# MAGPIE-ICL/synthPy

Hardware: AMD Instinct MI355X
Metric: ray-steps/sec (+ rays/sec to detector), 1e7 rays x 512^3 volume (higher is better)
Workload: dtype f64

## Files before the change

synthpy_amd/csrc/trace_tile.inc:

```
struct TileGeom {
  int tb, tc;
  int halo;
  int band;
};

struct TileArgs {
  TraceArgs A;
  TileGeom G;
  int k0, k1;
  int first, last;
  int exit_rec, slab;
  int rot;
  unsigned block0;
  const double *rec_in;
  const uint32_t *order;
  uint32_t *perm_out;
  double *strag_rec;
  int64_t strag_cap;
  unsigned long long *strag_count;
};

constexpr int kRecColD = (1024 + 80) / 8;
__host__ __device__ constexpr int tile_rec(bool aux, bool rec = false) { return aux ? 38 : (rec ? 16 : 18); }

__host__ __device__ inline size_t tile_lds_bytes(const TileGeom &g, int seg_steps, bool aux = false, bool rec = false) {
  const size_t tables = (size_t)(2 * (g.tb + 1) + 2 * (g.tc + 1) + 4);
  (void)seg_steps;
  const size_t head = rec ? (((tables * sizeof(double)) + 1023) & ~(size_t)1023) / sizeof(double) : ((tables + 1) & ~(size_t)1);
  if (rec) return sizeof(double) * (head + (size_t)5 * g.tc * kRecColD);
  return sizeof(double) * (head + (size_t)5 * g.tb * g.tc * tile_rec(aux, rec));
}

__device__ __forceinline__ uint32_t band_key(int ib, int ic, int ncc, int band) {
  const int bnd = ib / band, row = ib - bnd * band;
  const int col = (bnd & 1) ? ncc - 1 - ic : ic;
  return ((uint32_t)bnd * (uint32_t)ncc + (uint32_t)col) * (uint32_t)band + (uint32_t)row;
}

__global__ void k_keys_band(VolDev V, const double *__restrict__ s0, int64_t N, int axis, int band, uint32_t oob_key, int shift,
                            uint32_t *__restrict__ keys) {
  const int64_t i = blockIdx.x * (int64_t)blockDim.x + threadIdx.x;
  if (i >= N) return;
  const int b = (axis + 1) % 3, c = (axis + 2) % 3;
  double pa = s0[axis * N + i], pb = s0[b * N + i], pc = s0[c * N + i];
  const double va = s0[(3 + axis) * N + i], vb = s0[(3 + b) * N + i], vc = s0[(3 + c) * N + i];
  const double ga0 = V.g[0][0];
  if (va > 0 && pa < ga0) {
    const double tau = (ga0 - pa) / va;
    pb = pb + vb * tau;
    pc = pc + vc * tau;
  }
  const double gb0 = V.g[1][0], gbL = V.g[1][V.nb - 1], gc0 = V.g[2][0], gcL = V.g[2][V.nc - 1];
  uint32_t key = oob_key;
  if (pb >= gb0 && pb <= gbL && pc >= gc0 && pc <= gcL) {
    const int ib = find_cell(V.g[1], V.nb, pb, gb0, (V.nb - 1) / (gbL - gb0));
    const int ic = find_cell(V.g[2], V.nc, pc, gc0, (V.nc - 1) / (gcL - gc0));
    key = band_key(ib, ic, V.nc - 1, band) >> shift;
  }
  keys[i] = key;
}

__global__ void k_keys_band_rec(VolDev V, const double *__restrict__ rec, int64_t N, int band, uint32_t oob_key, int shift,
                                uint32_t *__restrict__ keys) {
  const int64_t j = blockIdx.x * (int64_t)blockDim.x + threadIdx.x;
  if (j >= N) return;
  const double pb = rec[j], pc = rec[N + j], va = rec[2 * N + j];
  const double gb0 = V.g[1][0], gbL = V.g[1][V.nb - 1], gc0 = V.g[2][0], gcL = V.g[2][V.nc - 1];
  uint32_t key = oob_key;
  if (va > 0 && pb >= gb0 && pb <= gbL && pc >= gc0 && pc <= gcL) {
    const int ib = find_cell(V.g[1], V.nb, pb, gb0, (V.nb - 1) / (gbL - gb0));
    const int ic = find_cell(V.g[2], V.nc, pc, gc0, (V.nc - 1) / (gcL - gc0));
    key = band_key(ib, ic, V.nc - 1, band) >> shift;
  }
  keys[j] = key;
}

__global__ void k_strag_snap(const unsigned long long *count, unsigned long long *snap, int q, unsigned long long *total) {
  const unsigned long long c = *count;
  snap[q + 1] = c;
  *total += c - snap[q];
}

struct StragFinish {
  TraceArgs A;
  const double *strag;
  int64_t cap;
  int exit_rec, slab;
};
__global__ __launch_bounds__(256) void k_strag_finish(StragFinish F) {
  const TraceArgs &A = F.A;
  const int64_t N = A.N;
  const int64_t j = blockIdx.x * (int64_t)blockDim.x + threadIdx.x;
  const bool gone = j < N && A.rec[2 * N + j] == -__builtin_inf();
  double y[9];
#pragma unroll
  for (int row = 0; row < 9; ++row) y[row] = __builtin_nan("");
  if (gone) {
    const int64_t g = (int64_t)A.rec[j];
#pragma unroll
    for (int row = 0; row < 9; ++row) y[row] = F.strag[row * F.cap + g];
  }
  if (F.exit_rec) {
    if (gone) {
#pragma unroll
      for (int row = 0; row < 9; ++row) A.rec[row * N + j] = y[row];
    }
    return;
  }
  const bool finished = gone && y[2] == y[2] && y[6] <= A.t_end;
  if (finished) {
    const double rem = A.t_end - y[6];
    write_outputs(A, j, fma(y[2], rem, A.V.g[0][A.V.na - 1]), fma(y[3], rem, y[0]), fma(y[4], rem, y[1]), y[2], y[3], y[4], y[5], y[7], y[8]);
  }
  if (F.slab) {
    if (gone && !finished) write_lost(A, j);
  } else {
    queue_push(A.out_count, A.out_list, gone && !finished, (uint32_t)j);
  }
}

template <bool PHASE>
__global__ __launch_bounds__(256) void k_build_records(VolDev V, double *__restrict__ R) {
  const int64_t cells = (int64_t)(V.nb - 1) * (V.nc - 1), total = cells * V.na;
  for (int64_t t = blockIdx.x * (int64_t)blockDim.x + threadIdx.x; t < total; t += (int64_t)gridDim.x * blockDim.x) {
    const int k = (int)(t / cells);
    const int64_t rem = t - (int64_t)k * cells;
    const int ic = (int)(rem / (V.nb - 1)), ib = (int)(rem - (int64_t)ic * (V.nb - 1));
    const int64_t q = col8(V, ib, ic) + koff(V, k), sc = kSC, sb = (int64_t)V.nc * 8;
    float4 v[4] = {V.P[q], V.P[q + sc], V.P[q + sb], V.P[q + sb + sc]};
    float l[4] = {0.f, 0.f, 0.f, 0.f};
    if (PHASE) {
      l[0] = V.L[q];
      l[1] = V.L[q + sc];
      l[2] = V.L[q + sb];
      l[3] = V.L[q + sb + sc];
    }
    CoefPlane p;
    coefs_from_corners<PHASE>(v, l, p);
    double2 *o = reinterpret_cast<double2 *>(R + t * 16);
    o[0] = make_double2(p.a[0], p.a[1]);
    o[1] = make_double2(p.a[2], p.a[3]);
    o[2] = make_double2(p.b[0], p.b[1]);
    o[3] = make_double2(p.b[2], p.b[3]);
    o[4] = make_double2(p.c[0], p.c[1]);
    o[5] = make_double2(p.c[2], p.c[3]);
    o[6] = make_double2(p.d[0], p.d[1]);
    o[7] = make_double2(p.d[2], p.d[3]);
  }
}

#ifndef SR_TILE_THREADS
#define SR_TILE_THREADS 256
#endif
#ifndef SR_TILE_WAVES
#define SR_TILE_WAVES 3
#endif
#ifndef SR_TILE_REC_WAVES
#define SR_TILE_REC_WAVES 4
#endif
template <bool PHASE, bool AUX = false, bool REC = false>
__global__ __launch_bounds__(SR_TILE_THREADS, AUX ? 2 : (REC ? SR_TILE_REC_WAVES : SR_TILE_WAVES)) void k_trace_tile(TileArgs T) {
  static_assert(!(AUX && REC), "the ready-made records hold the gradient fields only");
  constexpr int kTileRec = tile_rec(AUX, REC);
  extern __shared__ double lds[];
  const TraceArgs &A = T.A;
  const VolDev &V = A.V;
  const int TB = T.G.tb, TC = T.G.tc, NC = TB * TC;
  double *tgb = lds, *trb = tgb + (TB + 1), *tgc = trb + (TB + 1), *trc = tgc + (TC + 1);
  int *org = reinterpret_cast<int *>(trc + (TC + 1));
  const size_t tables = REC ? ((((size_t)(2 * (TB + 1) + 2 * (TC + 1) + 4) * sizeof(double)) + 1023) & ~(size_t)1023) / sizeof(double)
                            : ((size_t)(2 * (TB + 1) + 2 * (TC + 1) + 4) + 1) & ~(size_t)1;
  double *recs = lds + tables;
  const int slot_d = REC ? TC * kRecColD : NC * kTileRec;
  auto cell_off = [&](int b_, int c_) { return REC ? c_ * (kRecColD * 8) + b_ * 16 : (c_ * TB + b_) * kTileRec; };

  const unsigned chunk = gridDim.x / 8;
  const unsigned bid = (blockIdx.x % 8) * chunk + blockIdx.x / 8;
  const bool wg_live = bid < A.n_blocks;
  const int64_t j = (int64_t)(T.block0 + bid) * blockDim.x + threadIdx.x;
  const bool have = wg_live && j < A.N;
  const int64_t N = A.N;
  const int a = A.axis, b = (a + 1) % 3, c = (a + 2) % 3;
  int64_t i = 0;

  double y0 = 0, y1 = 0, y2 = 1, y3 = 0, y4 = 0, y5 = 0, y6 = 0, y7 = 0, y8 = 0;
  bool alive = false;
  auto from_s0 = [&](const TraceArgs &Q, int64_t ray, double &q0, double &q1, double &q2, double &q3, double &q4, double &q5, double &q6) -> bool {
    const double pa = Q.s0[a * N + ray];
    q0 = Q.s0[b * N + ray];
    q1 = Q.s0[c * N + ray];
    q2 = Q.s0[(3 + a) * N + ray];
    q3 = Q.s0[(3 + b) * N + ray];
    q4 = Q.s0[(3 + c) * N + ray];
    q5 = Q.s0[7 * N + ray];
    q6 = 0;
    const double ga0 = Q.V.g[0][0];
    bool ok = (q2 > 0) && (pa <= ga0);
    if (ok && pa < ga0) {
      const double tau = (ga0 - pa) / q2;
      if (tau >= Q.t_end) {
        ok = false;
      } else {
        q0 = q0 + q3 * tau;
        q1 = q1 + q4 * tau;
        q6 = tau;
      }
    }
    return ok;
  };
  if (T.first) {
    i = have ? (int64_t)A.perm[j] : 0;
    if (have) alive = from_s0(A, i, y0, y1, y2, y3, y4, y5, y6);
    if (AUX && have) {
      y7 = A.s0[6 * N + i];
      y8 = A.s0[8 * N + i];
    }
    if (!alive) y2 = 1;
  } else if (have) {
    const int64_t o = (int64_t)T.order[j];
    const double *R = T.rec_in;
    if (AUX) {
      y7 = R[7 * N + o];
      y8 = R[8 * N + o];
    } else {
      A.rec[7 * N + j] = R[7 * N + o];
      A.rec[8 * N + j] = R[8 * N + o];
    }
    y0 = R[o];
    y1 = R[N + o];
    y2 = R[2 * N + o];
    y3 = R[3 * N + o];
    y4 = R[4 * N + o];
    y5 = R[5 * N + o];
    y6 = R[6 * N + o];
    const double idx = R[9 * N + o];
    A.rec[9 * N + j] = idx;
    T.perm_out[j] = (uint32_t)idx;
    alive = y2 == y2;
  }
  const bool gone = have && !T.first && y2 == -__builtin_inf();
  alive = alive && (y0 == y0) && (y1 == y1) && (y3 == y3) && (y4 == y4) && (y5 == y5) && (y2 < 1e30) && (y2 > 1e-30);
  const bool entered = alive;

  int cb = 0, cc = 0, xb = 0, xc = 0;
  if (alive) {
    const double gb0 = V.g[1][0], gbL = V.g[1][V.nb - 1], gc0 = V.g[2][0], gcL = V.g[2][V.nc - 1];
    if (y0 >= gb0 && y0 < gbL && y1 >= gc0 && y1 < gcL) {
      const double rb0 = (V.nb - 1) / (gbL - gb0), rc0 = (V.nc - 1) / (gcL - gc0);
      cb = find_cell(V.g[1], V.nb, y0, gb0, rb0);
      cc = find_cell(V.g[2], V.nc, y1, gc0, rc0);
      const double dz = (V.g[0][T.k1] - V.g[0][T.k0]) / y2;
      const double eb = fmin(fmax(fma(y3, dz, y0), gb0), gbL), ec = fmin(fmax(fma(y4, dz, y1), gc0), gcL);
      xb = find_cell(V.g[1], V.nb, eb, gb0, rb0);
      xc = find_cell(V.g[2], V.nc, ec, gc0, rc0);
    } else {
      alive = false;
    }
  }
  if (threadIdx.x < 8) org[threadIdx.x] = (threadIdx.x & 2) ? -1 : 0x7fffffff;
  __syncthreads();
  if (alive) {
    atomicMin(&org[0], cb);
    atomicMin(&org[1], cc);
    atomicMax(&org[2], cb);
    atomicMax(&org[3], cc);
    atomicMin(&org[4], min(cb, xb));
    atomicMin(&org[5], min(cc, xc));
    atomicMax(&org[6], max(cb, xb));
    atomicMax(&org[7], max(cc, xc));
  }
  __syncthreads();
  auto place = [](int lo_e, int hi_e, int lo_x, int hi_x, int t, int cells) {
    if (hi_e < 0) return 0;
    int lo = lo_x, hi = hi_x;
    if (hi - lo + 1 > t) {
      lo = lo_e;
      hi = hi_e;
    }
    if (hi - lo + 1 > t) hi = lo + t - 1;
    return min(max(lo - (t - (hi - lo + 1)) / 2, 0), cells - t);
  };
  const int ob = place(org[0], org[2], org[4], org[6], TB, V.nb - 1), oc = place(org[1], org[3], org[5], org[7], TC, V.nc - 1);
  for (int t = threadIdx.x; t <= TB; t += blockDim.x) {
    tgb[t] = V.g[1][ob + t];
    trb[t] = t < TB ? V.rg[1][ob + t] : 0.0;
  }
  for (int t = threadIdx.x; t <= TC; t += blockDim.x) {
    tgc[t] = V.g[2][oc + t];
    trc[t] = t < TC ? V.rg[2][oc + t] : 0.0;
  }
  __syncthreads();
  int tb = cb - ob, tc = cc - oc;
  if (alive && !(tb >= 0 && tb < TB && tc >= 0 && tc < TC)) alive = false;
  if (!alive) tb = tc = 0;
  double lo_b = tgb[tb], r_b = trb[tb], lo_c = tgc[tc], r_c = trc[tc];
  int cell = cell_off(tb, tc);

  const int p_first = T.rot ? (int)((blockIdx.x >> 8) & 3u) * 64 : 0;
  const int p_lane = (int)((threadIdx.x + blockDim.x - (unsigned)p_first % blockDim.x) % blockDim.x);
  const bool producer = !REC && wg_live && p_lane < NC;
  const int pcell = producer ? p_lane * kTileRec : 0;
  const int64_t sc = kSC, sb = (int64_t)V.nc * 8;
  const int64_t pcol = producer ? col8(V, ob + p_lane % TB, oc + p_lane / TB) : 0;
  struct RawPlane {
    float4 v[4];
    float l[4];
  };
  auto issue_raw = [&](int k, RawPlane &r) {
    const int64_t ko = koff(V, k);
    const float4 *q = V.P + pcol + ko;
    r.v[0] = q[0];
    r.v[1] = q[sc];
    r.v[2] = q[sb];
    r.v[3] = q[sb + sc];
    r.l[0] = r.l[1] = r.l[2] = r.l[3] = 0.f;
    if (PHASE) {
      const float *l = V.L + pcol + ko;
      r.l[0] = l[0];
      r.l[1] = l[sc];
      r.l[2] = l[sb];
      r.l[3] = l[sb + sc];
    }
  };
  const int a_lane = (int)threadIdx.x - 64;
  const bool aproducer = AUX && wg_live && a_lane >= 0 && a_lane < NC;
  const int apcell = aproducer ? a_lane * kTileRec + 16 : 16;
  const int64_t apcol = aproducer ? col8(V, ob + a_lane % TB, oc + a_lane / TB) : 0;
  auto store_aux = [&](int slot, int off, const AuxPlane &p) {
    double2 *o = reinterpret_cast<double2 *>(recs + slot * slot_d + off);
    const double f[20] = {p.a[0], p.a[1], p.a[2], p.a[3], p.a[4], p.b[0], p.b[1], p.b[2], p.b[3], p.b[4],
                          p.c[0], p.c[1], p.c[2], p.c[3], p.c[4], p.d[0], p.d[1], p.d[2], p.d[3], p.d[4]};
#pragma unroll
    for (int q = 0; q < 10; ++q) o[q] = make_double2(f[2 * q], f[2 * q + 1]);
  };
  auto load_aux_rec = [&](int slot, int off, AuxPlane &p) {
    const double2 *o = reinterpret_cast<const double2 *>(recs + slot * slot_d + off);
    double f[20];
#pragma unroll
    for (int q = 0; q < 10; ++q) {
      const double2 t = o[q];
      f[2 * q] = t.x;
      f[2 * q + 1] = t.y;
    }
#pragma unroll
    for (int q = 0; q < 5; ++q) {
      p.a[q] = f[q];
      p.b[q] = f[5 + q];
      p.c[q] = f[10 + q];
      p.d[q] = f[15 + q];
    }
  };
  auto produce_aux = [&](const double (&u)[4][5], int dst, int prev, int mid) {
    AuxPlane p, q;
    aux_coefs(u, p);
    store_aux(dst, apcell, p);
    if (prev >= 0) {
      load_aux_rec(prev, apcell, q);
#pragma unroll
      for (int f = 0; f < 5; ++f) {
        q.a[f] += p.a[f];
        q.b[f] += p.b[f];
        q.c[f] += p.c[f];
        q.d[f] += p.d[f];
      }
      store_aux(mid, apcell, q);
    }
  };
  auto store_rec = [&](int slot, int off, const CoefPlane &p) {
    double2 *o = reinterpret_cast<double2 *>(recs + slot * slot_d + off);
    o[0] = make_double2(p.a[0], p.a[1]);
    o[1] = make_double2(p.a[2], p.a[3]);
    o[2] = make_double2(p.b[0], p.b[1]);
    o[3] = make_double2(p.b[2], p.b[3]);
    o[4] = make_double2(p.c[0], p.c[1]);
    o[5] = make_double2(p.c[2], p.c[3]);
    o[6] = make_double2(p.d[0], p.d[1]);
    o[7] = make_double2(p.d[2], p.d[3]);
  };
  auto load_rec = [&](int slot, int off, CoefPlane &p) {
    const double2 *q = reinterpret_cast<const double2 *>(recs + slot * slot_d + off);
    const double2 a01 = q[0], a23 = q[1], b01 = q[2], b23 = q[3], c01 = q[4], c23 = q[5], d01 = q[6], d23 = q[7];
    p.a[0] = a01.x; p.a[1] = a01.y; p.a[2] = a23.x; p.a[3] = a23.y;
    p.b[0] = b01.x; p.b[1] = b01.y; p.b[2] = b23.x; p.b[3] = b23.y;
    p.c[0] = c01.x; p.c[1] = c01.y; p.c[2] = c23.x; p.c[3] = c23.y;
    p.d[0] = d01.x; p.d[1] = d01.y; p.d[2] = d23.x; p.d[3] = d23.y;
  };
  auto produce = [&](const RawPlane &r, int dst, int prev, int mid) {
    CoefPlane p, q;
    coefs_from_corners<PHASE>(r.v, r.l, p);
    store_rec(dst, pcell, p);
    if (prev >= 0) {
      load_rec(prev, pcell, q);
#pragma unroll
      for (int f = 0; f < 4; ++f) {
        q.a[f] += p.a[f];
        q.b[f] += p.b[f];
        q.c[f] += p.c[f];
        q.d[f] += p.d[f];
      }
      store_rec(mid, pcell, q);
    }
  };
  const int wv = __builtin_amdgcn_readfirstlane((int)(threadIdx.x >> 6));
  const int ln = (int)(threadIdx.x & 63);
  const int ob_u = __builtin_amdgcn_readfirstlane(ob), oc_u = __builtin_amdgcn_readfirstlane(oc);
  const unsigned lane_off = (unsigned)(ln & 7) * 128u + (unsigned)(ln >> 3) * 16u;
  const int64_t col_bytes = (int64_t)(V.nb - 1) * 128, plane_bytes = (int64_t)(V.nc - 1) * col_bytes;
  const char *tile_r = REC ? reinterpret_cast<const char *>(V.R) + ((int64_t)oc_u * (V.nb - 1) + ob_u) * 128 : nullptr;
  const unsigned recs_lds = (unsigned)(uintptr_t)recs;
  auto slot_h = [&](int slot) { return REC ? (int)(recs_lds + (unsigned)(slot * slot_d) * 8u) : slot; };
  const int wcol_b = 2 * wv * (kRecColD * 8);
  const char *wcol_r = REC ? tile_r + (int64_t)(2 * wv) * col_bytes : nullptr;
  auto glds16 = [&](const char *src, int dst) { lds_dma16(src, lane_off, (unsigned)dst); };
  auto dma_cols = [&](const char *src0, const char *src1, int slot) {
    if (2 * wv < TC) glds16(src0, slot + wcol_b);
    if (2 * wv + 1 < TC) glds16(src1, slot + wcol_b + kRecColD * 8);
  };
  typedef double d2 __attribute__((ext_vector_type(2)));
  typedef __attribute__((address_space(3))) d2 *lds_d2_t;
  const int mid_lane = wcol_b + ln * 16;
  auto mid_from = [&](int lo, int hi, int mid, bool col0, bool col1) {
#pragma unroll
    for (int q = 0; q < 2; ++q) {
      if (!(q ? col1 : col0)) break;
      const d2 a = ((lds_d2_t)(uintptr_t)(unsigned)(lo + mid_lane))[q * (kRecColD / 2)];
      const d2 b = ((lds_d2_t)(uintptr_t)(unsigned)(hi + mid_lane))[q * (kRecColD / 2)];
      ((lds_d2_t)(uintptr_t)(unsigned)(mid + mid_lane))[q * (kRecColD / 2)] = a + b;
    }
  };
  if (REC && wg_live) {
    const char *p0 = wcol_r + (int64_t)T.k0 * plane_bytes;
    dma_cols(p0, p0 + col_bytes, slot_h(T.k0 % 3));
    dma_cols(p0 + plane_bytes, p0 + plane_bytes + col_bytes, slot_h((T.k0 + 1) % 3));
    asm volatile("s_waitcnt vmcnt(0)" ::: "memory");
    mid_from(slot_h(T.k0 % 3), slot_h((T.k0 + 1) % 3), slot_h(3 + T.k0 % 2), 2 * wv < TC, 2 * wv + 1 < TC);
  }
  if (producer) {
    RawPlane r0, r1;
    issue_raw(T.k0, r0);
    issue_raw(T.k0 + 1, r1);
    produce(r0, T.k0 % 3, -1, 0);
    produce(r1, (T.k0 + 1) % 3, T.k0 % 3, 3 + T.k0 % 2);
  }
  if (aproducer) {
    double u0[4][5], u1[4][5];
    aux_corners(V, apcol + koff(V, T.k0), u0);
    aux_corners(V, apcol + koff(V, T.k0 + 1), u1);
    produce_aux(u0, T.k0 % 3, -1, 0);
    produce_aux(u1, (T.k0 + 1) % 3, T.k0 % 3, 3 + T.k0 % 2);
  }
  __syncthreads();

#ifdef SR_TILE_EXP_NORELOC
  constexpr unsigned kInside = 0xFFFFFFFFu;
#else
  constexpr unsigned kInside = 0x3FEFFFFFu;
#endif
  auto relocate2 = [&](double qb, double qc, double wb, double wc) -> bool {
    const int nb_ = min(max(tb + (wb < 0.0 ? -1 : (hi_word(wb) >= kInside ? 1 : 0)), 0), TB - 1);
    const int nc_ = min(max(tc + (wc < 0.0 ? -1 : (hi_word(wc) >= kInside ? 1 : 0)), 0), TC - 1);
    double lb = tgb[nb_], ub = tgb[nb_ + 1], rb = trb[nb_], lc = tgc[nc_], uc = tgc[nc_ + 1], rc = trc[nc_];
    asm("" : "+v"(lb), "+v"(ub), "+v"(rb), "+v"(lc), "+v"(uc), "+v"(rc));
#ifdef SR_TILE_RELOC_SELECT
    bool in = true;
    if ((qb >= lb) & (qb < ub)) {
      tb = nb_;
      lo_b = lb;
      r_b = rb;
    } else {
      in = false;
    }
    if ((qc >= lc) & (qc < uc)) {
      tc = nc_;
      lo_c = lc;
      r_c = rc;
    } else {
      in = false;
    }
    return in;
#else
    tb = nb_;
    lo_b = lb;
    r_b = rb;
    tc = nc_;
    lo_c = lc;
    r_c = rc;
    return (qb >= lb) & (qb < ub) & (qc >= lc) & (qc < uc);
#endif
  };

  struct Rec {
    d2 q[8];
    int off;
  };
  auto request = [&](int slot, int cell_d, Rec &R) {
    R.off = REC ? 0 : slot * slot_d + cell_d;
    const unsigned addr = REC ? (unsigned)slot + (unsigned)cell_d : recs_lds + (unsigned)(slot * slot_d + cell_d) * 8u;
    if (REC)
      asm volatile("ds_read_b128 %0, %8\n\tds_read_b128 %1, %8 offset:128\n\tds_read_b128 %2, %8 offset:256\n\tds_read_b128 %3, %8 offset:384\n\t"
                   "ds_read_b128 %4, %8 offset:512\n\tds_read_b128 %5, %8 offset:640\n\tds_read_b128 %6, %8 offset:768\n\tds_read_b128 %7, %8 offset:896"
                   : "=&v"(R.q[0]), "=&v"(R.q[1]), "=&v"(R.q[2]), "=&v"(R.q[3]), "=&v"(R.q[4]), "=&v"(R.q[5]), "=&v"(R.q[6]), "=&v"(R.q[7])
                   : "v"(addr));
    else
      asm volatile("ds_read_b128 %0, %8\n\tds_read_b128 %1, %8 offset:16\n\tds_read_b128 %2, %8 offset:32\n\tds_read_b128 %3, %8 offset:48\n\t"
                   "ds_read_b128 %4, %8 offset:64\n\tds_read_b128 %5, %8 offset:80\n\tds_read_b128 %6, %8 offset:96\n\tds_read_b128 %7, %8 offset:112"
                   : "=&v"(R.q[0]), "=&v"(R.q[1]), "=&v"(R.q[2]), "=&v"(R.q[3]), "=&v"(R.q[4]), "=&v"(R.q[5]), "=&v"(R.q[6]), "=&v"(R.q[7])
                   : "v"(addr));
  };
#define SR_REC_WAIT(R, n)                                                                                                       \
  asm volatile("s_waitcnt lgkmcnt(" #n ")"                                                                                      \
               : "+v"(R.q[0]), "+v"(R.q[1]), "+v"(R.q[2]), "+v"(R.q[3]), "+v"(R.q[4]), "+v"(R.q[5]), "+v"(R.q[6]), "+v"(R.q[7]))

  int s_lo = slot_h(T.k0 % 3), s_hi = slot_h((T.k0 + 1) % 3), s_nx = slot_h((T.k0 + 2) % 3);
  int m_cur = slot_h(3 + T.k0 % 2), m_nx = slot_h(3 + (T.k0 + 1) % 2);
  constexpr int kNever = -0x7fffffff - 1;
  const int k_col0 = (wg_live && 2 * wv < TC) ? T.k1 - 2 : kNever, k_col1 = (wg_live && 2 * wv + 1 < TC) ? T.k1 - 2 : kNever;
  const char *nx_r0 = REC ? wcol_r + (int64_t)(T.k0 + 2) * plane_bytes : nullptr, *nx_r1 = REC ? nx_r0 + col_bytes : nullptr;
  Rec RA, RB;
  request(s_lo, cell, RA);
  typedef const double __attribute__((address_space(4))) *cdbl_t;
  const cdbl_t ctab = (cdbl_t)(uintptr_t)A.tab64;
  const cdbl_t tab0 = ctab + 8 * (int64_t)T.k0;
  cdbl_t tab = tab0;
  double nh = tab[0], nhh = tab[1], nh6 = tab[2], nh6w = tab[6];
  for (int k = T.k0; k < T.k1; ++k) {
    const double Sh = nh, Shh = nhh, Sh6 = nh6, Sh6w = nh6w;
    {
      tab = k + 1 < T.k1 ? tab + 8 : tab0;
      nh = tab[0];
      nhh = tab[1];
      nh6 = tab[2];
      nh6w = tab[6];
    }
    RawPlane NX;
    double NXU[20];
    const bool more = k + 2 <= T.k1;
    const bool more0 = k <= k_col0, more1 = k <= k_col1;
#ifndef SR_TILE_EXP_NOPRODUCE
    if (REC) {
      if (more0) glds16(nx_r0, s_nx + wcol_b);
      if (more1) glds16(nx_r1, s_nx + wcol_b + kRecColD * 8);
    } else if (!AUX) {
      if (producer && more) issue_raw(k + 2, NX);
    } else {
      if (producer && more) {
        RawPlane t;
        issue_raw(k + 2, t);
#pragma unroll
        for (int e = 0; e < 4; ++e) {
          NXU[2 * e] = __hiloint2double(__float_as_int(t.v[e].y), __float_as_int(t.v[e].x));
          NXU[2 * e + 1] = __hiloint2double(__float_as_int(t.v[e].w), __float_as_int(t.v[e].z));
        }
        NXU[8] = __hiloint2double(__float_as_int(t.l[1]), __float_as_int(t.l[0]));
        NXU[9] = __hiloint2double(__float_as_int(t.l[3]), __float_as_int(t.l[2]));
      }
      if (aproducer && more) {
        double u[4][5];
        aux_corners(V, apcol + koff(V, k + 2), u);
#pragma unroll
        for (int e = 0; e < 4; ++e)
#pragma unroll
          for (int f = 0; f < 5; ++f) NXU[5 * e + f] = u[e][f];
      }
    }
#endif
    if (alive) {
      double kp0, kp1, kv0, kv1, kv2, kph, iv;
      double ap0, ap1, av0, av1, av2, aph, at;
      double k7 = 0, k8 = 0, a7 = 0, a8 = 0;
      bool ok = true;
      double wb = (y0 - lo_b) * r_b, wc = (y1 - lo_c) * r_c;
      if (max(hi_word(wb), hi_word(wc)) >= kInside) {
        const int was = cell;
        if (!relocate2(y0, y1, wb, wc)) ok = false;
        cell = cell_off(tb, tc);
        wb = (y0 - lo_b) * r_b;
        wc = (y1 - lo_c) * r_c;
        if (cell != was) request(s_lo, cell, RA);
      }
      bool moved = false;
      auto stage = [&](auto SI, auto HASNEXT, double t2, double t3, double t4, double t7, Rec &R, Rec &NXT, int nslot, double &nwb, double &nwc) {
        constexpr int s = decltype(SI)::value;
        constexpr bool has_next = decltype(HASNEXT)::value;
        iv = s == 0 ? rcp_f64_from_f32(t2) : rcp_refine(t2, iv);
        const double p0 = t3 * iv, p1 = t4 * iv;
        if (s < 3) {
          const double w = s == 2 ? Sh : Shh;
          const double qb = fma(w, p0, y0), qc = fma(w, p1, y1);
          nwb = (qb - lo_b) * r_b;
          nwc = (qc - lo_c) * r_c;
          if (max(hi_word(nwb), hi_word(nwc)) >= kInside) {
            const int was = cell;
            if (!relocate2(qb, qc, nwb, nwc)) ok = false;
            cell = cell_off(tb, tc);
            moved = cell != was;
            nwb = (qb - lo_b) * r_b;
            nwc = (qc - lo_c) * r_c;
          }
          if (has_next) request(nslot, cell, NXT);
        }
        if (has_next)
          SR_REC_WAIT(R, 8);
        else
          SR_REC_WAIT(R, 0);
        double F[4];
        F[0] = fma(wc, fma3(wb, R.q[6].x, R.q[4].x), fma3(wb, R.q[2].x, R.q[0].x));
        F[1] = fma(wc, fma3(wb, R.q[6].y, R.q[4].y), fma3(wb, R.q[2].y, R.q[0].y));
        F[2] = fma(wc, fma3(wb, R.q[7].x, R.q[5].x), fma3(wb, R.q[3].x, R.q[1].x));
        F[3] = PHASE ? fma(wc, fma3(wb, R.q[7].y, R.q[5].y), fma3(wb, R.q[3].y, R.q[1].y)) : 0.0;
        const double ivf = (s == 1 || s == 2) ? iv * 0.5 : iv;
        double r7 = 0, r8 = 0;
        if (AUX) {
          AuxPlane P;
          load_aux_rec(0, R.off + 16, P);
          double X[5], damp, dpol;
          aux_eval(P, wb, wc, (s == 1 || s == 2) ? 0.5 : 1.0, X);
          aux_rates(V, a, X, t7, t2, t3, t4, damp, dpol);
          r7 = damp * iv;
          r8 = dpol * iv;
        }
        if (s == 0) {
          ap0 = p0;
          ap1 = p1;
          av0 = F[0] * ivf;
          av1 = F[1] * ivf;
          av2 = F[2] * ivf;
          at = iv;
          if (PHASE) aph = F[3] * ivf;
          if (AUX) {
            a7 = r7;
            a8 = r8;
          }
        } else {
          kp0 = p0;
          kp1 = p1;
          kv0 = F[0] * ivf;
          kv1 = F[1] * ivf;
          kv2 = F[2] * ivf;
          if (PHASE) kph = F[3] * ivf;
          if (AUX) {
            k7 = r7;
            k8 = r8;
          }
          if (s < 3) {
            ap0 = fma(2.0, kp0, ap0); ap1 = fma(2.0, kp1, ap1);
            av0 = fma(2.0, kv0, av0); av1 = fma(2.0, kv1, av1); av2 = fma(2.0, kv2, av2);
            at = fma(2.0, iv, at);
            if (PHASE) aph = fma(2.0, kph, aph);
            if (AUX) {
              a7 = fma(2.0, k7, a7);
              a8 = fma(2.0, k8, a8);
            }
          }
        }
      };
      double w1b, w1c, w2b, w2c, w3b, w3c;
      stage(std::integral_constant<int, 0>{}, std::true_type{}, y2, y3, y4, y7, RA, RB, m_cur, w1b, w1c);
      {
        const double t2 = fma(Shh, av2, y2), t3 = fma(Shh, av0, y3), t4 = fma(Shh, av1, y4);
        ok = ok && (t2 > 0);
        wb = w1b;
        wc = w1c;
        moved = false;
        stage(std::integral_constant<int, 1>{}, std::false_type{}, t2, t3, t4, AUX ? fma(Shh, a7, y7) : 0.0, RB, RB, 0, w2b, w2c);
        if (moved) request(m_cur, cell, RB);
      }
      {
        const double t2 = fma(Shh, kv2, y2), t3 = fma(Shh, kv0, y3), t4 = fma(Shh, kv1, y4);
        ok = ok && (t2 > 0);
        wb = w2b;
        wc = w2c;
        stage(std::integral_constant<int, 2>{}, std::true_type{}, t2, t3, t4, AUX ? fma(Shh, k7, y7) : 0.0, RB, RA, s_hi, w3b, w3c);
      }
      {
        const double t2 = fma(Sh, kv2, y2), t3 = fma(Sh, kv0, y3), t4 = fma(Sh, kv1, y4);
        ok = ok && (t2 > 0);
        wb = w3b;
        wc = w3c;
        double dummy0, dummy1;
        stage(std::integral_constant<int, 3>{}, std::false_type{}, t2, t3, t4, AUX ? fma(Sh, k7, y7) : 0.0, RA, RA, 0, dummy0, dummy1);
      }
      y0 = fma(Sh6, ap0 + kp0, y0);
      y1 = fma(Sh6, ap1 + kp1, y1);
      y2 = fma(Sh6, av2 + kv2, y2);
      y3 = fma(Sh6, av0 + kv0, y3);
      y4 = fma(Sh6, av1 + kv1, y4);
      if (PHASE) y5 = fma(Sh6w, aph + kph, y5);
      y6 = fma(Sh6, at + iv, y6);
      if (AUX) {
        y7 = fma(Sh6, a7 + k7, y7);
        y8 = fma(Sh6, a8 + k8, y8);
      }
      if (!ok || !(y2 > 0)) alive = false;
    }
#ifndef SR_TILE_EXP_NOPRODUCE
    if (REC) {
      if (more0) {
        asm volatile("s_waitcnt vmcnt(0)" ::: "memory");
        mid_from(s_hi, s_nx, m_nx, true, more1);
      }
    } else if (!AUX) {
      if (producer && more) produce(NX, s_nx, s_hi, m_nx);
    } else {
      if (producer && more) {
        RawPlane t;
#pragma unroll
        for (int e = 0; e < 4; ++e) {
          t.v[e].x = __int_as_float(__double2loint(NXU[2 * e]));
          t.v[e].y = __int_as_float(__double2hiint(NXU[2 * e]));
          t.v[e].z = __int_as_float(__double2loint(NXU[2 * e + 1]));
          t.v[e].w = __int_as_float(__double2hiint(NXU[2 * e + 1]));
        }
        t.l[0] = __int_as_float(__double2loint(NXU[8]));
        t.l[1] = __int_as_float(__double2hiint(NXU[8]));
        t.l[2] = __int_as_float(__double2loint(NXU[9]));
        t.l[3] = __int_as_float(__double2hiint(NXU[9]));
        produce(t, s_nx, s_hi, m_nx);
      }
      if (aproducer && more) {
        double u[4][5];
#pragma unroll
        for (int e = 0; e < 4; ++e)
#pragma unroll
          for (int f = 0; f < 5; ++f) u[e][f] = NXU[5 * e + f];
        produce_aux(u, s_nx, s_hi, m_nx);
      }
    }
#endif
#ifndef SR_TILE_EXP_NOBARRIER
    __syncthreads();
#endif
    if (REC) {
      nx_r0 += plane_bytes;
      nx_r1 += plane_bytes;
    }
    const int t = s_lo;
    s_lo = s_hi;
    s_hi = s_nx;
    s_nx = t;
    m_cur ^= m_nx;
    m_nx ^= m_cur;
    m_cur ^= m_nx;
  }
#undef SR_REC_WAIT

  const TileArgs *tail_args = (const TileArgs *)__builtin_amdgcn_kernarg_segment_ptr();
  asm volatile("" : "+s"(tail_args));
  const TraceArgs &B = tail_args->A;
  unsigned long long tot = 0;
  const bool lost = have && entered && !alive;
  {
    const unsigned long long mask = __ballot(lost);
    if (mask != 0ull) {
      const int lane = threadIdx.x & 63;
      const int leader = __ffsll((long long)mask) - 1;
      unsigned long long base = 0;
      if (lane == leader) base = atomicAdd(tail_args->strag_count, (unsigned long long)__popcll(mask));
      base = __shfl(base, leader, 64);
      if (lost) {
        const int64_t g = (int64_t)(base + (unsigned long long)__popcll(mask & ((1ull << lane) - 1ull)));
        double *S = tail_args->strag_rec;
        const int64_t cap = tail_args->strag_cap;
        if (tail_args->first) {
          double q0, q1, q2, q3, q4, q5, q6;
          from_s0(B, i, q0, q1, q2, q3, q4, q5, q6);
          S[g] = q0;
          S[cap + g] = q1;
          S[2 * cap + g] = q2;
          S[3 * cap + g] = q3;
          S[4 * cap + g] = q4;
          S[5 * cap + g] = q5;
          S[6 * cap + g] = q6;
          S[7 * cap + g] = B.s0[6 * N + i];
          S[8 * cap + g] = B.s0[8 * N + i];
          S[9 * cap + g] = (double)i;
        } else {
          const int64_t o = (int64_t)tail_args->order[j];
          const double *R = tail_args->rec_in;
#pragma unroll
          for (int row = 0; row < 10; ++row) S[row * cap + g] = R[row * N + o];
        }
        B.rec[j] = (double)g;
        B.rec[2 * N + j] = -__builtin_inf();
      }
    }
  }
  const bool to_rec = !tail_args->last || tail_args->exit_rec;
  if (have && tail_args->first) {
    B.rec[7 * N + j] = B.s0[6 * N + i];
    B.rec[8 * N + j] = B.s0[8 * N + i];
    B.rec[9 * N + j] = (double)i;
  }
  if (to_rec) {
    if (have && !lost) {
      const double nan = __builtin_nan("");
      const bool keep = alive || gone;
      if (AUX) {
        B.rec[7 * N + j] = keep ? y7 : nan;
        B.rec[8 * N + j] = keep ? y8 : nan;
      }
      B.rec[j] = keep ? y0 : nan;
      B.rec[N + j] = keep ? y1 : nan;
      B.rec[2 * N + j] = keep ? y2 : nan;
      B.rec[3 * N + j] = keep ? y3 : nan;
      B.rec[4 * N + j] = keep ? y4 : nan;
      B.rec[5 * N + j] = keep ? y5 : nan;
      B.rec[6 * N + j] = keep ? y6 : nan;
    }
    if (tail_args->last && alive) tot = (unsigned long long)(B.V.na - 1);
  } else {
    if (have && !lost) {
      B.rec[2 * N + j] = gone ? y2 : 0.0;
      if (gone) B.rec[j] = y0;
    }
    const bool finished = alive && y6 <= B.t_end;
    if (finished) {
      double amp = y7, pol = y8;
      if (!AUX) {
        if (tail_args->first) {
          amp = B.s0[6 * N + i];
          pol = B.s0[8 * N + i];
        } else {
          amp = B.rec[7 * N + j];
          pol = B.rec[8 * N + j];
        }
      }
      const double rem = B.t_end - y6;
      write_outputs(B, j, fma(y2, rem, B.V.g[0][B.V.na - 1]), fma(y3, rem, y0), fma(y4, rem, y1), y2, y3, y4, y5, amp, pol);
      tot = (unsigned long long)(B.V.na - 1);
    }
    if (tail_args->slab) {
      if (have && !finished && !lost && !gone) write_lost(B, j);
    } else {
      queue_push(B.out_count, B.out_list, have && !finished && !lost && !gone, (uint32_t)j);
    }
  }
  for (int off = 32; off > 0; off >>= 1) tot += __shfl_down(tot, off, 64);
  if ((threadIdx.x & 63) == 0 && tot) atomicAdd(sr::stripe(B.counters, B.step_stripe), tot);
}
```

Measured before the change: 121.9 billion.

## Pad cell-edge tables with sentinels and interleave them for branchless relocation

Rewrites the per-tile grid-edge and reciprocal-width tables in LDS as interleaved (edge, reciprocal) pairs, padded on both sides with infinity sentinel entries. Relocation can then step the cell index without clamping and fetch the bounds with a few hand-issued LDS reads. It also recomputes the fractional weights inside the relocation routine, derives the lower-bound test from the weight's sign bit, and pins some DMA operands in scalar and vector registers. This is meant to shorten the relocation path and reduce its register pressure. The risks are that out-of-tile steps now depend on the sentinel entries, and that the inline asm waits on every outstanding LDS operation.

```diff
diff --git a/synthpy_amd/csrc/trace_tile.inc b/synthpy_amd/csrc/trace_tile.inc
--- a/synthpy_amd/csrc/trace_tile.inc
+++ b/synthpy_amd/csrc/trace_tile.inc
@@ -23,8 +23,13 @@
 constexpr int kRecColD = (1024 + 80) / 8;
 __host__ __device__ constexpr int tile_rec(bool aux, bool rec = false) { return aux ? 38 : (rec ? 16 : 18); }
 
+constexpr int kTabLo = 4, kTabHi = 5;
+__host__ __device__ constexpr int tile_tab_entries(int t) { return kTabLo + t + kTabHi; }
+__host__ __device__ constexpr int tile_tab_doubles(int tb, int tc) { return 2 * tile_tab_entries(tb) + 2 * tile_tab_entries(tc) + 4; }
+static_assert(tile_tab_doubles(8, 8) * sizeof(double) <= 1024, "the records kernel's table head is one KiB");
+
 __host__ __device__ inline size_t tile_lds_bytes(const TileGeom &g, int seg_steps, bool aux = false, bool rec = false) {
-  const size_t tables = (size_t)(2 * (g.tb + 1) + 2 * (g.tc + 1) + 4);
+  const size_t tables = (size_t)(rec ? tile_tab_doubles(8, 8) : tile_tab_doubles(g.tb, g.tc));
   (void)seg_steps;
   const size_t head = rec ? (((tables * sizeof(double)) + 1023) & ~(size_t)1023) / sizeof(double) : ((tables + 1) & ~(size_t)1);
   if (rec) return sizeof(double) * (head + (size_t)5 * g.tc * kRecColD);
@@ -166,13 +171,14 @@
   const TraceArgs &A = T.A;
   const VolDev &V = A.V;
   const int TB = T.G.tb, TC = T.G.tc, NC = TB * TC;
-  double *tgb = lds, *trb = tgb + (TB + 1), *tgc = trb + (TB + 1), *trc = tgc + (TC + 1);
-  int *org = reinterpret_cast<int *>(trc + (TC + 1));
-  const size_t tables = REC ? ((((size_t)(2 * (TB + 1) + 2 * (TC + 1) + 4) * sizeof(double)) + 1023) & ~(size_t)1023) / sizeof(double)
-                            : ((size_t)(2 * (TB + 1) + 2 * (TC + 1) + 4) + 1) & ~(size_t)1;
+  const int tab_nb = tile_tab_entries(REC ? 8 : TB), tab_nc = tile_tab_entries(REC ? 8 : TC);
+  int *org = reinterpret_cast<int *>(lds + 2 * (tab_nb + tab_nc));
+  const size_t tables = REC ? 1024 / sizeof(double) : ((size_t)tile_tab_doubles(TB, TC) + 1) & ~(size_t)1;
+  const unsigned tab_b = (unsigned)(uintptr_t)(__attribute__((address_space(3))) double *)lds + kTabLo * 16u;
+  const unsigned tab_c = tab_b + (unsigned)tab_nb * 16u;
   double *recs = lds + tables;
   const int slot_d = REC ? TC * kRecColD : NC * kTileRec;
-  auto cell_off = [&](int b_, int c_) { return REC ? c_ * (kRecColD * 8) + b_ * 16 : (c_ * TB + b_) * kTileRec; };
+  auto cell_off = [&](int b_, int c_) { return REC ? __mul24(c_, kRecColD * 8) + b_ * 16 : (c_ * TB + b_) * kTileRec; };
 
   const unsigned chunk = gridDim.x / 8;
   const unsigned bid = (blockIdx.x % 8) * chunk + blockIdx.x / 8;
@@ -281,19 +287,31 @@
     return min(max(lo - (t - (hi - lo + 1)) / 2, 0), cells - t);
   };
   const int ob = place(org[0], org[2], org[4], org[6], TB, V.nb - 1), oc = place(org[1], org[3], org[5], org[7], TC, V.nc - 1);
-  for (int t = threadIdx.x; t <= TB; t += blockDim.x) {
-    tgb[t] = V.g[1][ob + t];
-    trb[t] = t < TB ? V.rg[1][ob + t] : 0.0;
-  }
-  for (int t = threadIdx.x; t <= TC; t += blockDim.x) {
-    tgc[t] = V.g[2][oc + t];
-    trc[t] = t < TC ? V.rg[2][oc + t] : 0.0;
-  }
+  typedef double d2 __attribute__((ext_vector_type(2)));
+  typedef __attribute__((address_space(3))) d2 *lds_d2_t;
+  auto fill_table = [&](unsigned tab, int t_cells, const double *g, const double *rg, int o) {
+    for (int t = threadIdx.x; t < tile_tab_entries(t_cells); t += blockDim.x) {
+      const int n = t - kTabLo;
+      d2 e = {n < 0 ? __builtin_inf() : -__builtin_inf(), 1.0};
+      if (n >= 0 && n <= t_cells) e.x = g[o + n];
+      if (n >= 0 && n < t_cells) e.y = rg[o + n];
+      ((lds_d2_t)(uintptr_t)tab)[n] = e;
+    }
+  };
+  fill_table(tab_b, TB, V.g[1], V.rg[1], ob);
+  fill_table(tab_c, TC, V.g[2], V.rg[2], oc);
   __syncthreads();
   int tb = cb - ob, tc = cc - oc;
   if (alive && !(tb >= 0 && tb < TB && tc >= 0 && tc < TC)) alive = false;
   if (!alive) tb = tc = 0;
-  double lo_b = tgb[tb], r_b = trb[tb], lo_c = tgc[tc], r_c = trc[tc];
+  double lo_b, r_b, lo_c, r_c;
+  {
+    const d2 eb = ((lds_d2_t)(uintptr_t)tab_b)[tb], ec = ((lds_d2_t)(uintptr_t)tab_c)[tc];
+    lo_b = eb.x;
+    r_b = eb.y;
+    lo_c = ec.x;
+    r_c = ec.y;
+  }
   int cell = cell_off(tb, tc);
 
   const int p_first = T.rot ? (int)((blockIdx.x >> 8) & 3u) * 64 : 0;
@@ -404,7 +422,7 @@
   const int wv = __builtin_amdgcn_readfirstlane((int)(threadIdx.x >> 6));
   const int ln = (int)(threadIdx.x & 63);
   const int ob_u = __builtin_amdgcn_readfirstlane(ob), oc_u = __builtin_amdgcn_readfirstlane(oc);
-  const unsigned lane_off = (unsigned)(ln & 7) * 128u + (unsigned)(ln >> 3) * 16u;
+  unsigned lane_off = (unsigned)(ln & 7) * 128u + (unsigned)(ln >> 3) * 16u;
   const int64_t col_bytes = (int64_t)(V.nb - 1) * 128, plane_bytes = (int64_t)(V.nc - 1) * col_bytes;
   const char *tile_r = REC ? reinterpret_cast<const char *>(V.R) + ((int64_t)oc_u * (V.nb - 1) + ob_u) * 128 : nullptr;
   const unsigned recs_lds = (unsigned)(uintptr_t)recs;
@@ -416,8 +434,6 @@
     if (2 * wv < TC) glds16(src0, slot + wcol_b);
     if (2 * wv + 1 < TC) glds16(src1, slot + wcol_b + kRecColD * 8);
   };
-  typedef double d2 __attribute__((ext_vector_type(2)));
-  typedef __attribute__((address_space(3))) d2 *lds_d2_t;
   const int mid_lane = wcol_b + ln * 16;
   auto mid_from = [&](int lo, int hi, int mid, bool col0, bool col1) {
 #pragma unroll
@@ -456,37 +472,19 @@
 #else
   constexpr unsigned kInside = 0x3FEFFFFFu;
 #endif
-  auto relocate2 = [&](double qb, double qc, double wb, double wc) -> bool {
-    const int nb_ = min(max(tb + (wb < 0.0 ? -1 : (hi_word(wb) >= kInside ? 1 : 0)), 0), TB - 1);
-    const int nc_ = min(max(tc + (wc < 0.0 ? -1 : (hi_word(wc) >= kInside ? 1 : 0)), 0), TC - 1);
-    double lb = tgb[nb_], ub = tgb[nb_ + 1], rb = trb[nb_], lc = tgc[nc_], uc = tgc[nc_ + 1], rc = trc[nc_];
-    asm("" : "+v"(lb), "+v"(ub), "+v"(rb), "+v"(lc), "+v"(uc), "+v"(rc));
-#ifdef SR_TILE_RELOC_SELECT
-    bool in = true;
-    if ((qb >= lb) & (qb < ub)) {
-      tb = nb_;
-      lo_b = lb;
-      r_b = rb;
-    } else {
-      in = false;
-    }
-    if ((qc >= lc) & (qc < uc)) {
-      tc = nc_;
-      lo_c = lc;
-      r_c = rc;
-    } else {
-      in = false;
-    }
-    return in;
-#else
-    tb = nb_;
-    lo_b = lb;
-    r_b = rb;
-    tc = nc_;
-    lo_c = lc;
-    r_c = rc;
-    return (qb >= lb) & (qb < ub) & (qc >= lc) & (qc < uc);
-#endif
+  auto relocate2 = [&](double qb, double qc, double &wb, double &wc) -> bool {
+    const int hb = (int)hi_word(wb), hc = (int)hi_word(wc);
+    tb += (hb >> 31) + (hb >= (int)kInside ? 1 : 0);
+    tc += (hc >> 31) + (hc >= (int)kInside ? 1 : 0);
+    const unsigned ab = tab_b + ((unsigned)tb << 4), ac = tab_c + ((unsigned)tc << 4);
+    double ub, uc;
+    asm volatile("ds_read_b64 %0, %6\n\tds_read_b64 %1, %6 offset:8\n\tds_read_b64 %2, %6 offset:16\n\t"
+                 "ds_read_b64 %3, %7\n\tds_read_b64 %4, %7 offset:8\n\tds_read_b64 %5, %7 offset:16\n\ts_waitcnt lgkmcnt(0)"
+                 : "=&v"(lo_b), "=&v"(r_b), "=&v"(ub), "=&v"(lo_c), "=&v"(r_c), "=&v"(uc)
+                 : "v"(ab), "v"(ac));
+    wb = (qb - lo_b) * r_b;
+    wc = (qc - lo_c) * r_c;
+    return ((int)max(hi_word(wb), hi_word(wc)) >= 0) & (qb < ub) & (qc < uc);
   };
 
   struct Rec {
@@ -538,8 +536,14 @@
     const bool more0 = k <= k_col0, more1 = k <= k_col1;
 #ifndef SR_TILE_EXP_NOPRODUCE
     if (REC) {
-      if (more0) glds16(nx_r0, s_nx + wcol_b);
-      if (more1) glds16(nx_r1, s_nx + wcol_b + kRecColD * 8);
+      if (more0) {
+        asm volatile("" : "+s"(nx_r0), "+v"(lane_off));
+        glds16(nx_r0, s_nx + wcol_b);
+      }
+      if (more1) {
+        asm volatile("" : "+s"(nx_r1), "+v"(lane_off));
+        glds16(nx_r1, s_nx + wcol_b + kRecColD * 8);
+      }
     } else if (!AUX) {
       if (producer && more) issue_raw(k + 2, NX);
     } else {
@@ -574,8 +578,6 @@
         const int was = cell;
         if (!relocate2(y0, y1, wb, wc)) ok = false;
         cell = cell_off(tb, tc);
-        wb = (y0 - lo_b) * r_b;
-        wc = (y1 - lo_c) * r_c;
         if (cell != was) request(s_lo, cell, RA);
       }
       bool moved = false;
@@ -594,8 +596,6 @@
             if (!relocate2(qb, qc, nwb, nwc)) ok = false;
             cell = cell_off(tb, tc);
             moved = cell != was;
-            nwb = (qb - lo_b) * r_b;
-            nwc = (qc - lo_c) * r_c;
           }
           if (has_next) request(nslot, cell, NXT);
         }
```

Result: faster. 124.4 billion, median of 6 (+2.1%).
